# Nick-qsv/MLP-PPO-2PLY-P3

Measured on AMD Instinct MI355X. Metric: self-play env steps/sec (whole node) + 2-ply evals/sec at batch=65536, higher is better.
Workload: dtype int8 boards / fp32-equivalent policy MLP (split-f16 MFMA); 1 GPU; C3: B=65536 games/GPU PPO rollout step (policy 198->128->{500,1} + masked sample + env.step, rollout rows stored to an HBM ring); global_batch=65536, games_per_gpu=65536, max_legal_moves=500, parallelism=dp1 (independent game shards), streams_per_gpu=4, step_fork=False

## Files before the change

mlp-ppo-2ply-p3_amd/csrc/bg_mlp.hip:

```cpp
#include <hip/hip_runtime.h>
#include <stdint.h>
#include <stdlib.h>
#include "bg_host.h"
#include "bg_debug.h"


namespace {

constexpr int kW1Ahead = 2;

typedef float f32x16 __attribute__((ext_vector_type(16)));
typedef _Float16 f16x8 __attribute__((ext_vector_type(8)));

constexpr int kIn = 198;
constexpr int kKB1 = (kIn + 15) / 16;
constexpr float kMaskLog = -103.27892990343185f;
constexpr int kHdr = 16;

__device__ __forceinline__ int lane_id() { return threadIdx.x & 63; }

__host__ __device__ inline int kperm_src(int kb, int h, int i) {
    if (kb < 12) {
        const int p = kb >= 6 ? 1 : 0;
        const int pt = 4 * (kb - 6 * p) + 2 * h + (i >> 2);
        return 98 * p + 4 * pt + (i & 3);
    }
    if (kb > 12 || h != 0 || i >= 6) return -1;
    return i < 2 ? 96 + i : 192 + i;
}

__device__ __forceinline__ f16x8 feats8(const uint8_t* rec, int kb, int h) {
    f16x8 f;
    if (kb < 12) {
        const int base = (kb >= 6 ? 24 + 4 * (kb - 6) : 4 * kb) + 2 * h;
        #pragma unroll
        for (int q = 0; q < 2; ++q) {
            const int n = rec[base + q];
            f[4 * q + 0] = n >= 1 ? (_Float16)1.0f : (_Float16)0.0f;
            f[4 * q + 1] = n >= 2 ? (_Float16)1.0f : (_Float16)0.0f;
            f[4 * q + 2] = n >= 3 ? (_Float16)1.0f : (_Float16)0.0f;
            f[4 * q + 3] = (_Float16)(n >= 3 ? (float)(n - 3) * 0.5f : 0.0f);
        }
    } else {
        const bool on = h == 0;
        f[0] = on ? (_Float16)((float)rec[48] * 0.5f) : (_Float16)0.0f;
        f[1] = on ? (_Float16)(float)rec[50] : (_Float16)0.0f;
        f[2] = on ? (_Float16)((float)rec[49] * 0.5f) : (_Float16)0.0f;
        f[3] = on ? (_Float16)(float)rec[51] : (_Float16)0.0f;
        f[4] = on && rec[52] == 0 ? (_Float16)1.0f : (_Float16)0.0f;
        f[5] = on && rec[52] != 0 ? (_Float16)1.0f : (_Float16)0.0f;
        f[6] = (_Float16)0.0f;
        f[7] = (_Float16)0.0f;
    }
    return f;
}

__device__ __forceinline__ void split(float x, _Float16& hi, _Float16& lo) {
    hi = (_Float16)x;
    lo = (_Float16)(x - (float)hi);
}

__device__ __forceinline__ f16x8 as_h8(uint4 v) { return __builtin_bit_cast(f16x8, v); }

__device__ __forceinline__ int scale_exp(float max_abs) {
    if (!(max_abs > 0.0f) || !(max_abs < INFINITY)) return 0;
    int q;
    (void)frexpf(max_abs, &q);
    const int e = 14 - q;
    return e < -100 ? -100 : (e > 100 ? 100 : e);
}

__device__ __forceinline__ uint32_t mix32(uint32_t x) {
    x ^= x >> 16; x *= 0x7FEB352Du; x ^= x >> 15; x *= 0x846CA68Bu; x ^= x >> 16;
    return x;
}

__device__ __forceinline__ float fast_ln(float x) { return __builtin_amdgcn_logf(x) * 0.69314718055994531f; }
__device__ __forceinline__ float fast_exp(float x) { return __builtin_amdgcn_exp2f(x * 1.4426950408889634f); }

constexpr float kGumbelMax = 17.0f;

__device__ __forceinline__ float gumbel(uint32_t w) {
    const float u = ((float)(w >> 9) + 0.5f) * (1.0f / 8388608.0f);
    const float v = 1.0f - u;
    const float series = v * (1.0f + v * (0.5f + v * (1.0f / 3.0f)));
    const float e = v < (1.0f / 64.0f) ? series : -fast_ln(u);
    return -fast_ln(e);
}

__device__ __forceinline__ int hid(int r, int h) { return (r & 3) + 8 * (r >> 2) + 4 * h; }

struct PackView {
    const int* hdr;
    const uint4* w1q;
    const float* b1p;
    const uint4* w2q;
    const float* b2p;
};

__host__ __device__ inline int sz_w1q(int T) { return kKB1 * T * 2 * 64 * 4; }
__host__ __device__ inline int sz_b1p(int T) { return T * 16 * 64; }
__host__ __device__ inline int sz_w2q(int T, int OT) { return OT * T * 2 * 2 * 64 * 4; }
__host__ __device__ inline int sz_b2p(int OT) { return OT * 16 * 64; }

template <typename P>
__host__ __device__ inline void views(P base, int T, int OT, P& hdr, P& w1q, P& b1p, P& w2q, P& b2p) {
    hdr = base;
    w1q = hdr + kHdr;
    b1p = w1q + sz_w1q(T);
    w2q = b1p + sz_b1p(T);
    b2p = w2q + sz_w2q(T, OT);
}

constexpr int kZWin = 256, kZCap = 64;
constexpr int kHeavyDefault = 64;
constexpr int kRowBestDefault = 2;

#ifdef BGX_POLICY_STAMPS
constexpr int kStampWaves = 8192;
__device__ unsigned long long g_pstamp[kStampWaves][6];
#define PSTAMP(k) do { if (MODE == 0 && sw < kStampWaves && lane_id() == 0) g_pstamp[sw][k] = __builtin_amdgcn_s_memrealtime(); } while (0)
#else
#define PSTAMP(k) do { } while (0)
#endif
constexpr float kSkipMargin = 30.0f;

template <int T, int MODE>
__global__ __launch_bounds__(MODE == 0 ? 256 : 64) __attribute__((amdgpu_waves_per_eu(2))) void k_policy_act(const uint8_t* __restrict__ recs, int n,
                                                   const float* __restrict__ packed, int n_actions, int n_otiles,
                                                   uint32_t seed_lo, uint32_t seed_hi, uint32_t step_arg,
                                                   const uint32_t* __restrict__ step_ctr, int greedy_arg,
                                                   int32_t* act_out, float* logp_out, float* value_out,
                                                   float* logits_arg, uint8_t* records_out, int skip_arg) {
#ifdef BGX_POLICY_STAMPS
    const int sw = (int)(blockIdx.x * (MODE == 0 ? 4 : 1) + (threadIdx.x >> 6));
#endif
    PSTAMP(0);
    const uint32_t step = step_arg + (step_ctr ? *step_ctr : 0u);
    constexpr int kW = MODE == 0 ? 4 : 1;
    const bool greedy = MODE < 0 ? (greedy_arg & 1) != 0 : false;
    const int rowbest = (greedy_arg >> 1) & 3;
    float* const logits_out = MODE < 0 ? logits_arg : nullptr;
    const bool skip_on = MODE == 0 && skip_arg != 0;
    __shared__ uint8_t srec_[kW][32 * 64];
    __shared__ int zl[MODE == 0 ? kZCap : 1];
    const float *hdrf, *w1f, *b1p, *w2f, *b2p;
    views(packed, T, n_otiles, hdrf, w1f, b1p, w2f, b2p);
    const uint4* w1q = (const uint4*)w1f;
    const uint4* w2q = (const uint4*)w2f;
    const int e1 = __builtin_bit_cast(int, hdrf[0]), e2 = __builtin_bit_cast(int, hdrf[1]);
    const int l = lane_id();
    const int j = l & 31, h = l >> 5;
    const int wv = kW > 1 ? __builtin_amdgcn_readfirstlane((int)(threadIdx.x >> 6)) : 0;
    uint8_t* const srec = srec_[wv];
    const int n_extra = skip_on ? 2 * ((n + kZWin - 1) / kZWin) : 0;
    const bool extra = (int)blockIdx.x < n_extra;
    const int row0 = (((int)blockIdx.x - n_extra) * kW + wv) * 32;
    if (!extra && row0 >= n) return;
    int nzw = 0;
    if (skip_on) {
        const int base = (extra ? (int)blockIdx.x >> 1 : row0 / kZWin) * kZWin;
        uint16_t cw[kZWin / 64];
        #pragma unroll
        for (int k = 0; k < kZWin / 64; ++k)
            cw[k] = *(const uint16_t*)(recs + (size_t)min(base + 64 * k + l, n - 1) * 64 + 60);
        #pragma unroll
        for (int k = 0; k < kZWin / 64; ++k) {
            const int r = base + 64 * k + l;
            const bool z = r < n && (cw[k] == 0 || (int)cw[k] > skip_arg);
            const uint64_t m = __ballot(z);
            const int pos = nzw + __popcll(m & ((1ull << l) - 1ull));
            if (extra && wv == 0 && z && pos < kZCap) zl[pos] = r;
            nzw += __popcll(m);
        }
    }
    const int kx = extra ? ((int)blockIdx.x & 1) : 0;
    const int nz = extra ? min(nzw - 32 * kx, 32) : 32;
    if (extra && (nzw > kZCap || nz <= 0)) return;
    const bool self_zero = skip_on && !extra && nzw > kZCap;
    const int vt = n_actions >> 5;
    if (extra) __syncthreads();
    {
        const int r = l >> 1, off = (l & 1) * 32;
        const int gr = extra ? zl[32 * kx + (r < nz ? r : 0)] : (row0 + r < n ? row0 + r : n - 1);
        const uint4* src = (const uint4*)(recs + (size_t)gr * 64 + off);
        uint4* dst = (uint4*)(srec + r * 64 + off);
        const uint4 v0 = src[0], v1 = src[1];
        dst[0] = v0;
        dst[1] = v1;
        if (!extra && records_out && row0 + r < n) {
            uint4* o = (uint4*)(records_out + (size_t)(row0 + r) * 64 + off);
            o[0] = v0;
            o[1] = v1;
        }
    }
    if (kW > 1) __builtin_amdgcn_wave_barrier(); else __syncthreads();
    const uint8_t* myrec = srec + j * 64;
    const int count = (int)myrec[60] | ((int)myrec[61] << 8);
    const bool gathered = skip_on && !extra && !self_zero && (count == 0 || count > skip_arg);
    const bool row_ok = extra ? j < nz : row0 + j < n;
    const int grow = extra ? zl[32 * kx + (j < nz ? j : 0)] : row0 + j;
    const int per = extra ? (n_otiles + kW - 1) / kW : n_otiles;
    const int o_beg = extra ? min(wv * per, n_otiles) : 0, o_end = extra ? min(o_beg + per, n_otiles) : n_otiles;

    PSTAMP(1);
    f32x16 x1[T];
    constexpr int kPD = kW1Ahead;
    if (kW > 1 && extra) {
        f32x16 acc;
        if (wv < T) {
            #pragma unroll
            for (int r = 0; r < 16; ++r) acc[r] = b1p[(wv * 16 + r) * 64 + l];
            uint4 wr[kPD + 1][2];
            #pragma unroll
            for (int p = 0; p < kPD; ++p)
                #pragma unroll
                for (int f = 0; f < 2; ++f) wr[p][f] = w1q[(p * 2 * T + 2 * wv + f) * 64 + l];
            #pragma unroll
            for (int kb = 0; kb < kKB1; ++kb) {
                if (kb + kPD < kKB1) {
                    #pragma unroll
                    for (int f = 0; f < 2; ++f)
                        wr[(kb + kPD) % (kPD + 1)][f] = w1q[((kb + kPD) * 2 * T + 2 * wv + f) * 64 + l];
                }
                __builtin_amdgcn_sched_barrier(0);
                const f16x8 bf = feats8(myrec, kb, h);
                acc = __builtin_amdgcn_mfma_f32_32x32x16_f16(as_h8(wr[kb % (kPD + 1)][1]), bf, acc, 0, 0, 0);
                acc = __builtin_amdgcn_mfma_f32_32x32x16_f16(as_h8(wr[kb % (kPD + 1)][0]), bf, acc, 0, 0, 0);
            }
        }
        float* const xs = (float*)&srec_[0][0];
        #pragma unroll
        for (int t0 = 0; t0 < T; t0 += 2) {
            __syncthreads();
            if (wv >= t0 && wv < t0 + 2 && wv < T) {
                #pragma unroll
                for (int r = 0; r < 16; ++r) xs[((wv - t0) * 16 + r) * 64 + l] = acc[r];
            }
            __syncthreads();
            #pragma unroll
            for (int t = t0; t < t0 + 2 && t < T; ++t)
                #pragma unroll
                for (int r = 0; r < 16; ++r) x1[t][r] = xs[((t - t0) * 16 + r) * 64 + l];
        }
    } else {
        #pragma unroll
        for (int t = 0; t < T; ++t)
            #pragma unroll
            for (int r = 0; r < 16; ++r) x1[t][r] = b1p[(t * 16 + r) * 64 + l];
        uint4 wf[kPD + 1][2 * T];
        #pragma unroll
        for (int p = 0; p < kPD; ++p)
            #pragma unroll
            for (int f = 0; f < 2 * T; ++f) wf[p][f] = w1q[(p * 2 * T + f) * 64 + l];
        #pragma unroll
        for (int kb = 0; kb < kKB1; ++kb) {
            if (kb + kPD < kKB1) {
                #pragma unroll
                for (int f = 0; f < 2 * T; ++f) wf[(kb + kPD) % (kPD + 1)][f] = w1q[((kb + kPD) * 2 * T + f) * 64 + l];
            }
            __builtin_amdgcn_sched_barrier(0);
            const f16x8 bf = feats8(myrec, kb, h);
            #pragma unroll
            for (int t = 0; t < T; ++t) {
                const f16x8 ah = as_h8(wf[kb % (kPD + 1)][2 * t + 0]);
                const f16x8 al = as_h8(wf[kb % (kPD + 1)][2 * t + 1]);
                x1[t] = __builtin_amdgcn_mfma_f32_32x32x16_f16(al, bf, x1[t], 0, 0, 0);
                x1[t] = __builtin_amdgcn_mfma_f32_32x32x16_f16(ah, bf, x1[t], 0, 0, 0);
            }
        }
    }
    float mx = 0.0f, hn2 = 0.0f;
    #pragma unroll
    for (int t = 0; t < T; ++t)
        #pragma unroll
        for (int r = 0; r < 16; ++r) {
            x1[t][r] = fmaxf(x1[t][r], 0.0f);
            mx = fmaxf(mx, x1[t][r]);
            if (skip_on) hn2 = fmaf(x1[t][r], x1[t][r], hn2);
        }
    #pragma unroll
    for (int d = 1; d < 64; d <<= 1) mx = fmaxf(mx, __shfl_xor(mx, d));
    int o_s = n_otiles;
    float ub = INFINITY;
    if (skip_on && !extra) {
        int cm = gathered ? 0 : count;
        #pragma unroll
        for (int d = 1; d < 32; d <<= 1) cm = max(cm, __shfl_xor(cm, d));
        o_s = max((cm + 31) >> 5, 1);
        hn2 += __shfl_xor(hn2, 32);
        const float u0 = hdrf[2] + hdrf[3] * ldexpf(sqrtf(hn2), -e1);
        ub = u0 + 1e-3f * fabsf(u0) + 1e-3f;
    }
    const int ex = scale_exp(mx);
    f16x8 xh[T][2], xl[T][2];
    #pragma unroll
    for (int t = 0; t < T; ++t)
        #pragma unroll
        for (int m = 0; m < 2; ++m)
            #pragma unroll
            for (int i = 0; i < 8; ++i) {
                _Float16 a, b;
                split(ldexpf(x1[t][8 * m + i], ex), a, b);
                xh[t][m][i] = a; xl[t][m][i] = b;
            }
    const int E = e2 + e1 + ex;
    const float up = ldexpf(1.0f, E), down = ldexpf(1.0f, -E);

    PSTAMP(2);
    float m = -INFINITY, s = 0.0f, best = -INFINITY, bestz = 0.0f, value = 0.0f;
    int besta = 0;
#ifdef BGX_POLICY_STAMPS
    unsigned long long ptiles = 0;
#endif
    const uint32_t rowkey = mix32(mix32(seed_lo ^ mix32(seed_hi + 0x9E3779B9u)) ^ step) ^ (uint32_t)grow * 0x85EBCA6Bu;
    constexpr int NF = T * 2 * 2;
    uint4 w[NF];
    float bq[16];
    if (o_beg < o_end) {
        #pragma unroll
        for (int f = 0; f < NF; ++f) w[f] = w2q[((size_t)o_beg * NF + f) * 64 + l];
        #pragma unroll
        for (int r = 0; r < 16; ++r) bq[r] = b2p[(o_beg * 16 + r) * 64 + l];
    } else {
        #pragma unroll
        for (int f = 0; f < NF; ++f) w[f] = make_uint4(0, 0, 0, 0);
        #pragma unroll
        for (int r = 0; r < 16; ++r) bq[r] = 0.0f;
    }
    for (int o = o_beg; o < o_end;) {
        f32x16 y;
        #pragma unroll
        for (int r = 0; r < 16; ++r) y[r] = bq[r] * up;
        #pragma unroll
        for (int t = 0; t < T; ++t)
            #pragma unroll
            for (int mm = 0; mm < 2; ++mm) {
                const f16x8 ah = as_h8(w[(t * 2 + mm) * 2 + 0]);
                const f16x8 al = as_h8(w[(t * 2 + mm) * 2 + 1]);
                y = __builtin_amdgcn_mfma_f32_32x32x16_f16(al, xh[t][mm], y, 0, 0, 0);
                y = __builtin_amdgcn_mfma_f32_32x32x16_f16(ah, xl[t][mm], y, 0, 0, 0);
                y = __builtin_amdgcn_mfma_f32_32x32x16_f16(ah, xh[t][mm], y, 0, 0, 0);
            }
        const bool at_s = o + 1 == o_s && o_s < vt;
        const int nx = at_s ? vt : o + 1;
        __asm__ volatile("" ::: "memory");
        if (nx < o_end) {
            #pragma unroll
            for (int f = 0; f < NF; ++f) w[f] = w2q[((size_t)nx * NF + f) * 64 + l];
        }
        float z[16];
        float tm = -INFINITY;
        #pragma unroll
        for (int r = 0; r < 16; ++r) {
            const int a = 32 * o + hid(r, h);
            const float z0 = y[r] * down;
            if (logits_out && row_ok && a <= n_actions) logits_out[(size_t)grow * (32 * n_otiles) + a] = z0;
            value = a == n_actions ? z0 : value;
            z[r] = a < n_actions ? (a < count ? z0 : z0 + kMaskLog) : -INFINITY;
            tm = fmaxf(tm, z[r]);
        }
        __asm__ volatile("" ::: "memory");
        if (nx < o_end) {
            #pragma unroll
            for (int r = 0; r < 16; ++r) bq[r] = b2p[(nx * 16 + r) * 64 + l];
        }
        const float mn = fmaxf(m, tm);
        if (mn != -INFINITY) {
            float acc = 0.0f;
            #pragma unroll
            for (int r = 0; r < 16; ++r) acc += fast_exp(z[r] - mn);
            s = s * fast_exp(m - mn) + acc;
            m = mn;
        }
        const float b_row = rowbest ? fmaxf(best, __shfl_xor(best, 32)) : best;
#ifdef BGX_POLICY_STAMPS
        bool drawn = false;
#endif
        #pragma unroll
        for (int g = 0; g < 4; ++g) {
            const float gm = !greedy && rowbest == 2
                ? fmaxf(fmaxf(z[4 * g], z[4 * g + 1]), fmaxf(z[4 * g + 2], z[4 * g + 3])) : tm;
            const bool draw = greedy ? gm > best : !(gm + kGumbelMax < fmaxf(b_row, best)) && !(rowbest && gathered);
#ifdef BGX_POLICY_STAMPS
            drawn = drawn || draw;
#endif
            if (draw) {
                #pragma unroll
                for (int r = 4 * g; r < 4 * g + 4; ++r) {
                    const int a = 32 * o + hid(r, h);
                    const float key = greedy ? z[r] : z[r] + gumbel(mix32(rowkey ^ ((uint32_t)a * 0xC2B2AE35u)));
                    const bool up_ = key > best;
                    best = up_ ? key : best;
                    besta = up_ ? a : besta;
                    bestz = up_ ? z[r] : bestz;
                }
            }
        }
#ifdef BGX_POLICY_STAMPS
        if (MODE == 0) {
            const unsigned long long any = __ballot(drawn) != 0ull;
            ptiles += 1ull + (any << 8);
            ptiles |= any && o == vt ? 1ull << 16 : 0ull;
            ptiles |= any && o >= o_s && o != vt ? 1ull << 17 : 0ull;
        }
#endif
        int next = o + 1;
        if (at_s) {
            const float m_row = fmaxf(m, __shfl_xor(m, 32)), b_row = fmaxf(best, __shfl_xor(best, 32));
            const bool ok = gathered || (ub + kMaskLog < m_row - kSkipMargin && ub + kMaskLog + kGumbelMax < b_row);
            if (__ballot(!ok) == 0ull) {
                next = vt;
            } else {
                int o1 = o + 1;
                __asm__ volatile("" : "+v"(o1));
                #pragma unroll
                for (int f = 0; f < NF; ++f) w[f] = w2q[((size_t)o1 * NF + f) * 64 + l];
                #pragma unroll
                for (int r = 0; r < 16; ++r) bq[r] = b2p[(o1 * 16 + r) * 64 + l];
            }
        }
        o = next;
    }
    if (kW > 1 && extra) {
        __shared__ float pm[kW > 1 ? kW - 1 : 1][5][64];
        __shared__ int pa[kW > 1 ? kW - 1 : 1][64];
        if (wv > 0) {
            pm[wv - 1][0][l] = m; pm[wv - 1][1][l] = s; pm[wv - 1][2][l] = best; pm[wv - 1][3][l] = bestz;
            pm[wv - 1][4][l] = value; pa[wv - 1][l] = besta;
        }
        __syncthreads();
        if (wv > 0) return;
        #pragma unroll
        for (int q = 0; q < kW - 1; ++q) {
            const float mq = pm[q][0][l], sq = pm[q][1][l], bq = pm[q][2][l], zq = pm[q][3][l];
            const int aq = pa[q][l];
            const float mn = fmaxf(m, mq);
            if (mn != -INFINITY) s = s * fast_exp(m - mn) + sq * fast_exp(mq - mn);
            m = mn;
            const bool tk = bq > best || (bq == best && aq < besta);
            best = tk ? bq : best;
            besta = tk ? aq : besta;
            bestz = tk ? zq : bestz;
            value += pm[q][4][l];
        }
    }
    PSTAMP(3);
#ifdef BGX_POLICY_STAMPS
    if (MODE == 0 && sw < kStampWaves && lane_id() == 0) {
        g_pstamp[sw][4] = extra ? 1 : 2;
        g_pstamp[sw][5] = ptiles;
    }
#endif
    const float m2 = __shfl_xor(m, 32), s2 = __shfl_xor(s, 32);
    const float best2 = __shfl_xor(best, 32), bestz2 = __shfl_xor(bestz, 32);
    const int besta2 = __shfl_xor(besta, 32);
    const float value2 = __shfl_xor(value, 32);
    const float mm = fmaxf(m, m2);
    const float ss = s * fast_exp(m - mm) + s2 * fast_exp(m2 - mm);
    const bool take2 = best2 > best || (best2 == best && besta2 < besta);
    const int a_fin = take2 ? besta2 : besta;
    const float z_fin = take2 ? bestz2 : bestz;
    const float v_fin = h == 0 ? value + value2 : 0.0f;
    if (h == 0 && row_ok && !gathered) {
        act_out[grow] = a_fin;
        if (logp_out) logp_out[grow] = fminf(fmaxf(z_fin - (mm + logf(ss)), -15.942384719848633f),
                                             -1.1920930376163597e-07f);
        if (value_out) value_out[grow] = v_fin;
    }
}

__global__ __launch_bounds__(1024) void k_policy_scale(const float* W1, const float* Wa, const float* ba,
                                                       const float* wv, int H, int A, float* hdr) {
    __shared__ float r1[16], r2[16], r3[16], r4[16];
    const int t = threadIdx.x;
    float m1 = 0.0f, m2 = 0.0f, bmax = -INFINITY, nmax = 0.0f;
    for (int i = t; i < H * kIn; i += 1024) m1 = fmaxf(m1, fabsf(W1[i]));
    for (int i = t; i < A * H; i += 1024) m2 = fmaxf(m2, fabsf(Wa[i]));
    for (int i = t; i < H; i += 1024) m2 = fmaxf(m2, fabsf(wv[i]));
    for (int a = t; a < A; a += 1024) {
        double q = 0.0;
        for (int k = 0; k < H; ++k) q += (double)Wa[(size_t)a * H + k] * (double)Wa[(size_t)a * H + k];
        nmax = fmaxf(nmax, (float)sqrt(q));
        bmax = fmaxf(bmax, ba[a]);
    }
    #pragma unroll
    for (int d = 1; d < 64; d <<= 1) {
        m1 = fmaxf(m1, __shfl_xor(m1, d)); m2 = fmaxf(m2, __shfl_xor(m2, d));
        bmax = fmaxf(bmax, __shfl_xor(bmax, d)); nmax = fmaxf(nmax, __shfl_xor(nmax, d));
    }
    if ((t & 63) == 0) { r1[t >> 6] = m1; r2[t >> 6] = m2; r3[t >> 6] = bmax; r4[t >> 6] = nmax; }
    __syncthreads();
    if (t == 0) {
        for (int w = 1; w < 16; ++w) {
            m1 = fmaxf(m1, r1[w]); m2 = fmaxf(m2, r2[w]); bmax = fmaxf(bmax, r3[w]); nmax = fmaxf(nmax, r4[w]);
        }
        hdr[0] = __builtin_bit_cast(float, scale_exp(m1));
        hdr[1] = __builtin_bit_cast(float, scale_exp(m2));
        hdr[2] = bmax;
        hdr[3] = nmax * (1.0f + 1.0f / 1024.0f);
        for (int i = 4; i < kHdr; ++i) hdr[i] = 0.0f;
    }
}

__global__ void k_policy_pack(const float* W1, const float* b1, const float* Wa, const float* ba, const float* wv,
                              const float* bv, int H, int A, int T, int OT, float* packed) {
    float *hdr, *w1f, *b1p, *w2f, *b2p;
    views(packed, T, OT, hdr, w1f, b1p, w2f, b2p);
    const int e1 = __builtin_bit_cast(int, hdr[0]), e2 = __builtin_bit_cast(int, hdr[1]);
    _Float16* w1h = (_Float16*)w1f;
    _Float16* w2h = (_Float16*)w2f;
    const int tid = blockIdx.x * blockDim.x + threadIdx.x;
    const int n1 = kKB1 * T * 64 * 8, nb1 = T * 16 * 64, n2 = OT * T * 2 * 64 * 8, nb2 = OT * 16 * 64;
    auto W2 = [&](int o, int k) -> float {
        if (k >= H) return 0.0f;
        if (o < A) return Wa[(size_t)o * H + k];
        if (o == A) return wv[k];
        return 0.0f;
    };
    auto B2 = [&](int o) -> float { return o < A ? ba[o] : (o == A ? bv[0] : 0.0f); };
    if (tid < n1) {
        const int i = tid % 8, l = (tid / 8) % 64, t = (tid / 512) % T, kb = tid / (512 * T);
        const int hrow = 32 * t + (l & 31), k = kperm_src(kb, l >> 5, i);
        const float wk = hrow < H && k >= 0 ? W1[(size_t)hrow * kIn + k] : 0.0f;
        const float w = ldexpf(k == 97 || k == 195 ? wk / 15.0f : wk, e1);
        _Float16 a, b;
        split(w, a, b);
        w1h[(((kb * T + t) * 2 + 0) * 64 + l) * 8 + i] = a;
        w1h[(((kb * T + t) * 2 + 1) * 64 + l) * 8 + i] = b;
    } else if (tid < n1 + nb1) {
        const int q = tid - n1;
        const int l = q % 64, r = (q / 64) % 16, t = q / (64 * 16);
        const int hrow = 32 * t + hid(r, l >> 5);
        b1p[q] = hrow < H ? ldexpf(b1[hrow], e1) : 0.0f;
    } else if (tid < n1 + nb1 + n2) {
        const int q = tid - n1 - nb1;
        const int i = q % 8, l = (q / 8) % 64, mm = (q / 512) % 2, t = (q / 1024) % T, o = q / (1024 * T);
        const int k = 32 * t + hid(8 * mm + i, l >> 5);
        _Float16 a, b;
        split(ldexpf(W2(32 * o + (l & 31), k), e2), a, b);
        const size_t f = (((size_t)(o * T + t) * 2 + mm) * 2) * 64 + l;
        w2h[f * 8 + i] = a;
        w2h[(f + 64) * 8 + i] = b;
    } else if (tid < n1 + nb1 + n2 + nb2) {
        const int q = tid - n1 - nb1 - n2;
        const int l = q % 64, r = (q / 64) % 16, o = q / (64 * 16);
        b2p[q] = B2(32 * o + hid(r, l >> 5));
    }
}


__constant__ static const float kOffDiv15[16] = {
    0.0f / 15.0f, 1.0f / 15.0f, 2.0f / 15.0f, 3.0f / 15.0f, 4.0f / 15.0f, 5.0f / 15.0f,
    6.0f / 15.0f, 7.0f / 15.0f, 8.0f / 15.0f, 9.0f / 15.0f, 10.0f / 15.0f, 11.0f / 15.0f,
    12.0f / 15.0f, 13.0f / 15.0f, 14.0f / 15.0f, 15.0f / 15.0f};

__global__ void k_fc1_pack(const _Float16* __restrict__ w1h, int hidden, int T, uint4* __restrict__ out) {
    const int g = blockIdx.x * blockDim.x + threadIdx.x;
    if (g >= kKB1 * T * 64) return;
    const int l = g & 63, t = (g >> 6) % T, kb = (g >> 6) / T;
    const int u = 32 * t + (l & 31);
    f16x8 v;
    #pragma unroll
    for (int i = 0; i < 8; ++i) {
        const int src = kperm_src(kb, l >> 5, i);
        v[i] = (u < hidden && src >= 0) ? w1h[(size_t)u * kIn + src] : (_Float16)0.0f;
    }
    out[g] = __builtin_bit_cast(uint4, v);
}

template <int T>
__global__ __launch_bounds__(512) __attribute__((amdgpu_waves_per_eu(4))) void k_fc1_rec(const uint8_t* __restrict__ recs, int n,
                                                  const uint4* __restrict__ w1f, const _Float16* __restrict__ b1h,
                                                  int hidden, _Float16* __restrict__ hout, float* __restrict__ hmax2) {
    __shared__ uint4 sw[kKB1 * T * 64];
    __shared__ __attribute__((aligned(16))) uint8_t srec[8][32 * 64];
    __shared__ float sb[32 * T];
    for (int i = threadIdx.x; i < kKB1 * T * 64; i += blockDim.x) sw[i] = w1f[i];
    for (int i = threadIdx.x; i < 32 * T; i += blockDim.x) sb[i] = i < hidden ? (float)b1h[i] : 0.0f;
    __syncthreads();
    const int l = lane_id(), wv = threadIdx.x >> 6;
    const int j = l & 31, h = l >> 5;
    const int ntiles = (n + 31) / 32, stride = gridDim.x * 8;
    int tile = blockIdx.x * 8 + wv;
    __shared__ float swm[8];
    float hm = 0.0f;
    const int r = l >> 1, off = (l & 1) * 32;
    uint4 v0 = make_uint4(0, 0, 0, 0), v1 = v0;
    if (tile < ntiles) {
        const int gr = tile * 32 + r < n ? tile * 32 + r : n - 1;
        const uint4* src = (const uint4*)(recs + (size_t)gr * 64 + off);
        v0 = src[0];
        v1 = src[1];
    }
    for (; tile < ntiles; tile += stride) {
        const int row0 = tile * 32;
        uint4* dst = (uint4*)(srec[wv] + r * 64 + off);
        dst[0] = v0;
        dst[1] = v1;
        __builtin_amdgcn_wave_barrier();
        if (tile + stride < ntiles) {
            const int nr = (tile + stride) * 32 + r;
            const uint4* src = (const uint4*)(recs + (size_t)(nr < n ? nr : n - 1) * 64 + off);
            v0 = src[0];
            v1 = src[1];
        }
        const uint8_t* myrec = srec[wv] + j * 64;
        f32x16 acc[T];
        #pragma unroll
        for (int t = 0; t < T; ++t)
            #pragma unroll
            for (int q = 0; q < 16; ++q) acc[t][q] = 0.0f;
        #pragma unroll
        for (int kb = 0; kb < kKB1; ++kb) {
            f16x8 bf = feats8(myrec, kb, h);
            if (kb == 12) {
                bf[1] = h == 0 ? (_Float16)kOffDiv15[myrec[50] & 15] : (_Float16)0.0f;
                bf[3] = h == 0 ? (_Float16)kOffDiv15[myrec[51] & 15] : (_Float16)0.0f;
            }
            #pragma unroll
            for (int t = 0; t < T; ++t)
                acc[t] = __builtin_amdgcn_mfma_f32_32x32x16_f16(as_h8(sw[(kb * T + t) * 64 + l]), bf, acc[t], 0, 0, 0);
        }
        __builtin_amdgcn_wave_barrier();
        float ss = 0.0f;
        typedef _Float16 h4 __attribute__((ext_vector_type(4)));
        if (hidden % 8 == 0) {
            _Float16* orow = hout + (size_t)(row0 + j) * hidden;
            #pragma unroll
            for (int t = 0; t < T; ++t)
                #pragma unroll
                for (int p = 0; p < 2; ++p) {
                    h4 v[2];
                    #pragma unroll
                    for (int e = 0; e < 2; ++e) {
                        const int q = 2 * p + e, u = 32 * t + 8 * q + 4 * h;
                        #pragma unroll
                        for (int i = 0; i < 4; ++i) {
                            v[e][i] = (_Float16)fmaxf(acc[t][4 * q + i] + sb[u + i], 0.0f);
                            if (u < hidden) ss = fmaf((float)v[e][i], (float)v[e][i], ss);
                        }
                    }
                    const uint2 a = __builtin_bit_cast(uint2, v[0]), b = __builtin_bit_cast(uint2, v[1]);
                    const auto s0 = __builtin_amdgcn_permlane32_swap(a.x, b.x, false, false);
                    const auto s1 = __builtin_amdgcn_permlane32_swap(a.y, b.y, false, false);
                    const int u8 = 32 * t + 8 * (2 * p + h);
                    if (row0 + j < n && u8 < hidden)
                        *(uint4*)(orow + u8) = make_uint4(s0[0], s1[0], s0[1], s1[1]);
                }
        } else if (row0 + j < n) {
            _Float16* orow = hout + (size_t)(row0 + j) * hidden;
            #pragma unroll
            for (int t = 0; t < T; ++t)
                #pragma unroll
                for (int q = 0; q < 4; ++q) {
                    const int u = 32 * t + 8 * q + 4 * h;
                    if (u < hidden) {
                        h4 v;
                        #pragma unroll
                        for (int i = 0; i < 4; ++i) {
                            v[i] = (_Float16)fmaxf(acc[t][4 * q + i] + sb[u + i], 0.0f);
                            ss = fmaf((float)v[i], (float)v[i], ss);
                        }
                        *(h4*)(orow + u) = v;
                    }
                }
        }
        if (row0 + j >= n) ss = 0.0f;
        hm = fmaxf(hm, ss + __shfl_xor(ss, 32));
    }
    if (hmax2) {
        #pragma unroll
        for (int o = 16; o > 0; o >>= 1) hm = fmaxf(hm, __shfl_xor(hm, o));
        if (l == 0) swm[wv] = hm;
        __syncthreads();
        if (threadIdx.x == 0) {
            float m = swm[0];
            for (int w = 1; w < 8; ++w) m = fmaxf(m, swm[w]);
            atomicMax((int*)hmax2, __float_as_int(m));
        }
    }
}

struct EpochPrep {
    const float *w1, *b1, *wa, *ba, *wv, *bv;
    int hidden, n_actions, T;
    uint4* w1pack;
    _Float16 *b1h, *w2h, *b2h;
    float *gw1, *gw2, *gb2, *hmax2;
    float* bound;
    double* sums;
};
__global__ __launch_bounds__(256) void k_ppo_epoch_prep(EpochPrep a) {
    const int H = a.hidden, A = a.n_actions;
    if (a.bound) {
        const int r = blockIdx.x * 4 + (threadIdx.x >> 6), l = threadIdx.x & 63;
        if (r < A) {
            float s = 0.0f;
            for (int c = l; c < H; c += 64) {
                const float v = (float)(_Float16)a.wa[(size_t)r * H + c];
                s = fmaf(v, v, s);
            }
            #pragma unroll
            for (int o = 32; o >= 1; o >>= 1) s += __shfl_xor(s, o);
            if (l == 0) {
                a.bound[r] = sqrtf(s);
                a.bound[512 + r] = fabsf((float)(_Float16)a.ba[r]);
            }
        }
    }
    const long long n0 = (long long)kKB1 * a.T * 64, n1 = n0 + H, n2 = n1 + 512LL * H, n3 = n2 + 512,
                    n4 = n3 + (long long)H * 208, n5 = n4 + 512LL * H, n6 = n5 + 512, n7 = n6 + 1;
    for (long long g = (long long)blockIdx.x * 256 + threadIdx.x; g < n7; g += (long long)gridDim.x * 256) {
        if (g < n0) {
            const int l = (int)(g & 63), t = (int)((g >> 6) % a.T), kb = (int)((g >> 6) / a.T);
            const int u = 32 * t + (l & 31);
            f16x8 v;
            #pragma unroll
            for (int i = 0; i < 8; ++i) {
                const int src = kperm_src(kb, l >> 5, i);
                v[i] = (u < H && src >= 0) ? (_Float16)a.w1[(size_t)u * kIn + src] : (_Float16)0.0f;
            }
            a.w1pack[g] = __builtin_bit_cast(uint4, v);
        } else if (g < n1) {
            const int u = (int)(g - n0);
            a.b1h[u] = (_Float16)a.b1[u];
        } else if (g < n2) {
            const long long e = g - n1;
            const int r = (int)(e / H), c = (int)(e % H);
            a.w2h[e] = r < A ? (_Float16)a.wa[(size_t)r * H + c] : (r == A ? (_Float16)a.wv[c] : (_Float16)0.0f);
        } else if (g < n3) {
            const int r = (int)(g - n2);
            a.b2h[r] = r < A ? (_Float16)a.ba[r] : (r == A ? (_Float16)a.bv[0] : (_Float16)0.0f);
        } else if (g < n4) {
            a.gw1[g - n3] = 0.0f;
        } else if (g < n5) {
            a.gw2[g - n4] = 0.0f;
        } else if (g < n6) {
            a.gb2[g - n5] = 0.0f;
        } else if (a.hmax2) {
            a.hmax2[0] = 0.0f;
        }
    }
    if (a.sums && blockIdx.x == 0 && threadIdx.x < 3) a.sums[threadIdx.x] = 0.0;
}

__global__ void k_counter_add(uint32_t* ctr, uint32_t v) {
    if (threadIdx.x == 0) *ctr += v;
}

}

extern "C" {

int bgx_policy_packed_size(int32_t hidden, int32_t n_actions) {
    if (hidden <= 0 || hidden > 128 || n_actions <= 0) return BGX_EINVAL;
    const int T = (hidden + 31) / 32, OT = (n_actions + 1 + 31) / 32;
    return kHdr + sz_w1q(T) + sz_b1p(T) + sz_w2q(T, OT) + sz_b2p(OT);
}

int bgx_policy_pack(const float* W1, const float* b1, const float* Wa, const float* ba, const float* wv, const float* bv,
                    int32_t hidden, int32_t n_actions, float* packed, void* stream) {
    const int total = bgx_policy_packed_size(hidden, n_actions);
    if (total < 0 || !W1 || !b1 || !Wa || !ba || !wv || !bv || !packed) return BGX_EINVAL;
    const int T = (hidden + 31) / 32, OT = (n_actions + 1 + 31) / 32;
    hipStream_t s = (hipStream_t)stream;
    hipLaunchKernelGGL(k_policy_scale, dim3(1), dim3(1024), 0, s, W1, Wa, ba, wv, hidden, n_actions, packed);
    const int work = kKB1 * T * 64 * 8 + T * 16 * 64 + OT * T * 2 * 64 * 8 + OT * 16 * 64;
    hipLaunchKernelGGL(k_policy_pack, dim3((work + 255) / 256), dim3(256), 0, s, W1, b1, Wa, ba, wv, bv, hidden,
                       n_actions, T, OT, packed);
    return bgx_launch_status();
}

#ifdef BGX_POLICY_STAMPS
extern "C" int bgx_debug_policy_stamps(unsigned long long* out, int32_t waves) {
    if (hipDeviceSynchronize() != hipSuccess) return BGX_EDEVICE;
    if (hipMemcpyFromSymbol(out, HIP_SYMBOL(g_pstamp), (size_t)(waves < kStampWaves ? waves : kStampWaves) * 48) != hipSuccess)
        return BGX_EDEVICE;
    static unsigned long long z[kStampWaves][6];
    return hipMemcpyToSymbol(HIP_SYMBOL(g_pstamp), z, sizeof z) == hipSuccess ? BGX_OK : BGX_EDEVICE;
}
#endif

int bgx_policy_act_ctr(const uint8_t* records_dev, int32_t n, const float* packed, int32_t hidden, int32_t n_actions,
                       uint64_t seed, uint32_t step, const uint32_t* step_ctr, int32_t greedy, int32_t* act_out,
                       float* logp_out, float* value_out, float* logits_out, uint8_t* records_out, void* stream) {
    if (bgx_policy_packed_size(hidden, n_actions) < 0 || n < 0 || (n > 0 && (!records_dev || !packed || !act_out)))
        return BGX_EINVAL;
    if (n == 0) return BGX_OK;
    const int T = (hidden + 31) / 32, OT = (n_actions + 1 + 31) / 32;
    const int n_main = (n + 31) / 32;
    const dim3 grid(n_main), blk(64);
    const int n_wg = (n + 127) / 128;
    hipStream_t s = (hipStream_t)stream;
    const uint32_t lo = (uint32_t)seed, hi = (uint32_t)(seed >> 32);
    const bool plain = !greedy && !logits_out;
    const bool skip = bgx_dbg_int("BGX_POLICY_SKIP", 1) != 0;
    const int heavy = (int)bgx_dbg_int("BGX_POLICY_HEAVY", kHeavyDefault);
    const int garg = (greedy ? 1 : 0) | ((int)min(max(bgx_dbg_int("BGX_POLICY_ROWBEST", kRowBestDefault), 0ll), 2ll) << 1);
    const dim3 grid0(skip ? n_wg + 2 * ((n + kZWin - 1) / kZWin) : n_wg);
#define BGX_ACT(TT)                                                                                           \
    do {                                                                                                      \
        if (plain)                                                                                            \
            hipLaunchKernelGGL((k_policy_act<TT, 0>), grid0, dim3(256), 0, s, records_dev, n, packed, n_actions, OT, \
                               lo, hi, step, step_ctr, garg, act_out, logp_out, value_out, logits_out,     \
                               records_out, skip ? (heavy > 0 ? heavy : 1) : 0);                             \
        else                                                                                                  \
            hipLaunchKernelGGL((k_policy_act<TT, -1>), grid, blk, 0, s, records_dev, n, packed, n_actions, OT,   \
                               lo, hi, step, step_ctr, garg, act_out, logp_out, value_out, logits_out,     \
                               records_out, 0);                                                               \
    } while (0)
    switch (T) {
        case 1: BGX_ACT(1); break;
        case 2: BGX_ACT(2); break;
        case 3: BGX_ACT(3); break;
        default: BGX_ACT(4); break;
    }
#undef BGX_ACT
    return bgx_launch_status();
}

int bgx_policy_act_rec(const uint8_t* records_dev, int32_t n, const float* packed, int32_t hidden, int32_t n_actions,
                       uint64_t seed, uint32_t step, int32_t greedy, int32_t* act_out, float* logp_out,
                       float* value_out, float* logits_out, uint8_t* records_out, void* stream) {
    return bgx_policy_act_ctr(records_dev, n, packed, hidden, n_actions, seed, step, nullptr, greedy, act_out, logp_out,
                              value_out, logits_out, records_out, stream);
}

int bgx_counter_add(uint32_t* ctr_dev, uint32_t v, void* stream) {
    if (!ctr_dev) return BGX_EINVAL;
    hipLaunchKernelGGL(k_counter_add, dim3(1), dim3(64), 0, (hipStream_t)stream, ctr_dev, v);
    return bgx_launch_status();
}

int bgx_policy_act(const uint8_t* records_dev, int32_t n, const float* packed, int32_t hidden, int32_t n_actions,
                   uint64_t seed, uint32_t step, int32_t greedy, int32_t* act_out, float* logp_out, float* value_out,
                   float* logits_out, void* stream) {
    return bgx_policy_act_rec(records_dev, n, packed, hidden, n_actions, seed, step, greedy, act_out, logp_out,
                              value_out, logits_out, nullptr, stream);
}

int bgx_fc1_packed_size(int32_t hidden) {
    if (hidden <= 0 || hidden > 128 || hidden % 4) return BGX_EINVAL;
    return kKB1 * ((hidden + 31) / 32) * 64 * 16;
}

int bgx_fc1_pack(const void* w1h_dev, int32_t hidden, void* packed_dev, void* stream) {
    if (bgx_fc1_packed_size(hidden) < 0 || !w1h_dev || !packed_dev) return BGX_EINVAL;
    if ((uintptr_t)packed_dev % 16) return BGX_EINVAL;
    const int T = (hidden + 31) / 32, work = kKB1 * T * 64;
    hipLaunchKernelGGL(k_fc1_pack, dim3((work + 255) / 256), dim3(256), 0, (hipStream_t)stream,
                       (const _Float16*)w1h_dev, hidden, T, (uint4*)packed_dev);
    return bgx_launch_status();
}

int bgx_ppo_epoch_prep(const float* w1_dev, const float* b1_dev, const float* wa_dev, const float* ba_dev,
                       const float* wv_dev, const float* bv_dev, int32_t hidden, int32_t n_actions, void* w1pack_dev,
                       void* b1h_dev, void* w2h_dev, void* b2h_dev, float* gw1_dev, float* gw2_dev, float* gb2_dev,
                       float* hmax2_dev_or_null, float* bound_dev_or_null, double* sums_dev_or_null, void* stream) {
    if (bgx_fc1_packed_size(hidden) < 0 || n_actions <= 0 || n_actions >= 512) return BGX_EINVAL;
    if (!w1_dev || !b1_dev || !wa_dev || !ba_dev || !wv_dev || !bv_dev || !w1pack_dev || !b1h_dev || !w2h_dev ||
        !b2h_dev || !gw1_dev || !gw2_dev || !gb2_dev || (uintptr_t)w1pack_dev % 16)
        return BGX_EINVAL;
    EpochPrep a{w1_dev, b1_dev, wa_dev, ba_dev, wv_dev, bv_dev, hidden, n_actions, (hidden + 31) / 32,
                (uint4*)w1pack_dev, (_Float16*)b1h_dev, (_Float16*)w2h_dev, (_Float16*)b2h_dev, gw1_dev, gw2_dev,
                gb2_dev, hmax2_dev_or_null, bound_dev_or_null, sums_dev_or_null};
    hipLaunchKernelGGL(k_ppo_epoch_prep, dim3(512), dim3(256), 0, (hipStream_t)stream, a);
    return bgx_launch_status();
}

int bgx_fc1_records(const uint8_t* records_dev, int32_t n, const void* packed_dev, const void* b1h_dev,
                    int32_t hidden, void* h_dev, void* stream) {
    return bgx_fc1_records_ex(records_dev, n, packed_dev, b1h_dev, hidden, h_dev, nullptr, stream);
}

int bgx_fc1_records_ex(const uint8_t* records_dev, int32_t n, const void* packed_dev, const void* b1h_dev,
                       int32_t hidden, void* h_dev, float* hmax2_dev, void* stream) {
    if (bgx_fc1_packed_size(hidden) < 0 || n < 0 || (n > 0 && (!records_dev || !packed_dev || !b1h_dev || !h_dev)))
        return BGX_EINVAL;
    if (((uintptr_t)records_dev | (uintptr_t)packed_dev) % 16 || (uintptr_t)h_dev % 8) return BGX_EINVAL;
    if (n == 0) return BGX_OK;
    const int T = (hidden + 31) / 32;
    const int tiles8 = (n + 255) / 256;
    const dim3 grid(tiles8 < 512 ? tiles8 : 512), blk(512);
    hipStream_t s = (hipStream_t)stream;
    const uint4* w = (const uint4*)packed_dev;
    const _Float16* b = (const _Float16*)b1h_dev;
    _Float16* o = (_Float16*)h_dev;
    switch (T) {
        case 1: hipLaunchKernelGGL((k_fc1_rec<1>), grid, blk, 0, s, records_dev, n, w, b, hidden, o, hmax2_dev); break;
        case 2: hipLaunchKernelGGL((k_fc1_rec<2>), grid, blk, 0, s, records_dev, n, w, b, hidden, o, hmax2_dev); break;
        case 3: hipLaunchKernelGGL((k_fc1_rec<3>), grid, blk, 0, s, records_dev, n, w, b, hidden, o, hmax2_dev); break;
        default: hipLaunchKernelGGL((k_fc1_rec<4>), grid, blk, 0, s, records_dev, n, w, b, hidden, o, hmax2_dev); break;
    }
    return bgx_launch_status();
}

}
```

Measured before the change: 552.4 million env steps/s.

## Sort policy rows by legal-move count and stop after value tile when skipping

```diff
diff --git a/mlp-ppo-2ply-p3_amd/csrc/bg_mlp.hip b/mlp-ppo-2ply-p3_amd/csrc/bg_mlp.hip
--- a/mlp-ppo-2ply-p3_amd/csrc/bg_mlp.hip
+++ b/mlp-ppo-2ply-p3_amd/csrc/bg_mlp.hip
@@ -115,10 +115,13 @@
 constexpr int kZWin = 256, kZCap = 64;
 constexpr int kHeavyDefault = 64;
 constexpr int kRowBestDefault = 2;
+constexpr int kSortDefault = 1;
+constexpr int kVTileDefault = 1;
 
 #ifdef BGX_POLICY_STAMPS
 constexpr int kStampWaves = 8192;
-__device__ unsigned long long g_pstamp[kStampWaves][6];
+constexpr int kStampSlots = 8;
+__device__ unsigned long long g_pstamp[kStampWaves][kStampSlots];
 #define PSTAMP(k) do { if (MODE == 0 && sw < kStampWaves && lane_id() == 0) g_pstamp[sw][k] = __builtin_amdgcn_s_memrealtime(); } while (0)
 #else
 #define PSTAMP(k) do { } while (0)
@@ -140,10 +143,13 @@
     constexpr int kW = MODE == 0 ? 4 : 1;
     const bool greedy = MODE < 0 ? (greedy_arg & 1) != 0 : false;
     const int rowbest = (greedy_arg >> 1) & 3;
+    const bool vtile = MODE == 0 && (greedy_arg & 8) != 0;
     float* const logits_out = MODE < 0 ? logits_arg : nullptr;
     const bool skip_on = MODE == 0 && skip_arg != 0;
+    const bool sort_on = skip_on && (greedy_arg & 16) != 0;
     __shared__ uint8_t srec_[kW][32 * 64];
     __shared__ int zl[MODE == 0 ? kZCap : 1];
+    __shared__ int prm_[kW][MODE == 0 ? 32 : 1];
     const float *hdrf, *w1f, *b1p, *w2f, *b2p;
     views(packed, T, n_otiles, hdrf, w1f, b1p, w2f, b2p);
     const uint4* w1q = (const uint4*)w1f;
@@ -158,8 +164,9 @@
     const int row0 = (((int)blockIdx.x - n_extra) * kW + wv) * 32;
     if (!extra && row0 >= n) return;
     int nzw = 0;
+    uint64_t mA[kZWin / 64] = {}, mB[kZWin / 64] = {};
+    const int base = (extra ? (int)blockIdx.x >> 1 : row0 / kZWin) * kZWin;
     if (skip_on) {
-        const int base = (extra ? (int)blockIdx.x >> 1 : row0 / kZWin) * kZWin;
         uint16_t cw[kZWin / 64];
         #pragma unroll
         for (int k = 0; k < kZWin / 64; ++k)
@@ -172,6 +179,11 @@
             const int pos = nzw + __popcll(m & ((1ull << l) - 1ull));
             if (extra && wv == 0 && z && pos < kZCap) zl[pos] = r;
             nzw += __popcll(m);
+            if (sort_on && !extra) {
+                const bool a = r < n && cw[k] != 0 && (int)cw[k] <= min(32, skip_arg);
+                mA[k] = __ballot(a);
+                mB[k] = __ballot(r < n && !z && !a);
+            }
         }
     }
     const int kx = extra ? ((int)blockIdx.x & 1) : 0;
@@ -179,17 +191,40 @@
     if (extra && (nzw > kZCap || nz <= 0)) return;
     const bool self_zero = skip_on && !extra && nzw > kZCap;
     const int vt = n_actions >> 5;
+    const bool sorted = sort_on && !extra && !self_zero;
+    int* const prm = prm_[wv];
+    int nrows = 32;
+    if (sorted) {
+        int nA = 0, nB = 0;
+        #pragma unroll
+        for (int k = 0; k < kZWin / 64; ++k) { nA += __popcll(mA[k]); nB += __popcll(mB[k]); }
+        const int p0 = row0 - base;
+        nrows = min(nA + nB - p0, 32);
+        if (nrows <= 0) return;
+        int pa = 0, pb = nA;
+        #pragma unroll
+        for (int k = 0; k < kZWin / 64; ++k) {
+            const uint64_t lt = (1ull << l) - 1ull;
+            const bool a = (mA[k] >> l) & 1ull, b = (mB[k] >> l) & 1ull;
+            const int p = (a ? pa + __popcll(mA[k] & lt) : pb + __popcll(mB[k] & lt)) - p0;
+            if ((a || b) && p >= 0 && p < 32) prm[p] = base + 64 * k + l;
+            pa += __popcll(mA[k]);
+            pb += __popcll(mB[k]);
+        }
+        __builtin_amdgcn_wave_barrier();
+    }
     if (extra) __syncthreads();
     {
         const int r = l >> 1, off = (l & 1) * 32;
-        const int gr = extra ? zl[32 * kx + (r < nz ? r : 0)] : (row0 + r < n ? row0 + r : n - 1);
+        const int gr = extra ? zl[32 * kx + (r < nz ? r : 0)]
+                             : sorted ? prm[r < nrows ? r : 0] : (row0 + r < n ? row0 + r : n - 1);
         const uint4* src = (const uint4*)(recs + (size_t)gr * 64 + off);
         uint4* dst = (uint4*)(srec + r * 64 + off);
         const uint4 v0 = src[0], v1 = src[1];
         dst[0] = v0;
         dst[1] = v1;
-        if (!extra && records_out && row0 + r < n) {
-            uint4* o = (uint4*)(records_out + (size_t)(row0 + r) * 64 + off);
+        if (records_out && (extra ? sort_on && wv == 0 && r < nz : sorted ? r < nrows : row0 + r < n)) {
+            uint4* o = (uint4*)(records_out + (size_t)gr * 64 + off);
             o[0] = v0;
             o[1] = v1;
         }
@@ -198,8 +233,8 @@
     const uint8_t* myrec = srec + j * 64;
     const int count = (int)myrec[60] | ((int)myrec[61] << 8);
     const bool gathered = skip_on && !extra && !self_zero && (count == 0 || count > skip_arg);
-    const bool row_ok = extra ? j < nz : row0 + j < n;
-    const int grow = extra ? zl[32 * kx + (j < nz ? j : 0)] : row0 + j;
+    const bool row_ok = extra ? j < nz : sorted ? j < nrows : row0 + j < n;
+    const int grow = extra ? zl[32 * kx + (j < nz ? j : 0)] : sorted ? prm[j < nrows ? j : 0] : row0 + j;
     const int per = extra ? (n_otiles + kW - 1) / kW : n_otiles;
     const int o_beg = extra ? min(wv * per, n_otiles) : 0, o_end = extra ? min(o_beg + per, n_otiles) : n_otiles;
 
@@ -328,7 +363,11 @@
         #pragma unroll
         for (int r = 0; r < 16; ++r) bq[r] = 0.0f;
     }
+    bool vonly = false;
     for (int o = o_beg; o < o_end;) {
+#ifdef BGX_POLICY_STAMPS
+        if (o == vt) PSTAMP(7);
+#endif
         f32x16 y;
         #pragma unroll
         for (int r = 0; r < 16; ++r) y[r] = bq[r] * up;
@@ -342,6 +381,14 @@
                 y = __builtin_amdgcn_mfma_f32_32x32x16_f16(ah, xl[t][mm], y, 0, 0, 0);
                 y = __builtin_amdgcn_mfma_f32_32x32x16_f16(ah, xh[t][mm], y, 0, 0, 0);
             }
+        if (vonly) {
+            #pragma unroll
+            for (int r = 0; r < 16; ++r) value = 32 * o + hid(r, h) == n_actions ? y[r] * down : value;
+#ifdef BGX_POLICY_STAMPS
+            ptiles += 1ull | 1ull << 18;
+#endif
+            break;
+        }
         const bool at_s = o + 1 == o_s && o_s < vt;
         const int nx = at_s ? vt : o + 1;
         __asm__ volatile("" ::: "memory");
@@ -411,6 +458,7 @@
             const bool ok = gathered || (ub + kMaskLog < m_row - kSkipMargin && ub + kMaskLog + kGumbelMax < b_row);
             if (__ballot(!ok) == 0ull) {
                 next = vt;
+                vonly = vtile && !self_zero;
             } else {
                 int o1 = o + 1;
                 __asm__ volatile("" : "+v"(o1));
@@ -420,6 +468,9 @@
                 for (int r = 0; r < 16; ++r) bq[r] = b2p[(o1 * 16 + r) * 64 + l];
             }
         }
+#ifdef BGX_POLICY_STAMPS
+        if (o == o_beg) PSTAMP(6);
+#endif
         o = next;
     }
     if (kW > 1 && extra) {
@@ -775,9 +826,9 @@
 #ifdef BGX_POLICY_STAMPS
 extern "C" int bgx_debug_policy_stamps(unsigned long long* out, int32_t waves) {
     if (hipDeviceSynchronize() != hipSuccess) return BGX_EDEVICE;
-    if (hipMemcpyFromSymbol(out, HIP_SYMBOL(g_pstamp), (size_t)(waves < kStampWaves ? waves : kStampWaves) * 48) != hipSuccess)
+    if (hipMemcpyFromSymbol(out, HIP_SYMBOL(g_pstamp), (size_t)(waves < kStampWaves ? waves : kStampWaves) * kStampSlots * 8) != hipSuccess)
         return BGX_EDEVICE;
-    static unsigned long long z[kStampWaves][6];
+    static unsigned long long z[kStampWaves][kStampSlots];
     return hipMemcpyToSymbol(HIP_SYMBOL(g_pstamp), z, sizeof z) == hipSuccess ? BGX_OK : BGX_EDEVICE;
 }
 #endif
@@ -797,7 +848,9 @@
     const bool plain = !greedy && !logits_out;
     const bool skip = bgx_dbg_int("BGX_POLICY_SKIP", 1) != 0;
     const int heavy = (int)bgx_dbg_int("BGX_POLICY_HEAVY", kHeavyDefault);
-    const int garg = (greedy ? 1 : 0) | ((int)min(max(bgx_dbg_int("BGX_POLICY_ROWBEST", kRowBestDefault), 0ll), 2ll) << 1);
+    const int garg = (greedy ? 1 : 0) | ((int)min(max(bgx_dbg_int("BGX_POLICY_ROWBEST", kRowBestDefault), 0ll), 2ll) << 1) |
+                     (bgx_dbg_int("BGX_POLICY_VTILE", kVTileDefault) != 0 ? 8 : 0) |
+                     (bgx_dbg_int("BGX_POLICY_SORT", kSortDefault) != 0 ? 16 : 0);
     const dim3 grid0(skip ? n_wg + 2 * ((n + kZWin - 1) / kZWin) : n_wg);
 #define BGX_ACT(TT)                                                                                           \
     do {                                                                                                      \
```

After: 558.9 million env steps/s (median of 6 runs). 1.2% higher.
